# oletizi/ol_dsp

Hardware: AMD Instinct MI355X
Metric: stereo samples/s across N effect instances @48kHz; % HBM roofline; 1/2/4/8 GPU (higher is better)
Workload: dtype f32; 1 GPU; chorus; instances_per_gpu=65536, instances_total=65536, block=256, parallelism=instance-shard x1 (no data-path collective)

## Files before the change

### ol_dsp_amd/csrc/chorus_stage_rf.h

```cpp
#pragma once
#include "chorus_stage_l.h"

namespace olfx {
namespace ch {

__device__ __forceinline__ float psv_direct(Rsrc rP, uint32_t pb, uint32_t pmask, uint64_t acc, uint32_t tau,
                                            uint32_t wi, uint32_t wf, uint32_t pmaxu) {
    const uint32_t ph = hi32(acc);
    float gA, gB;
    win_gains(unit24(ph), gA, gB);
    uint32_t di; float fr;
    pitch_split(ph, wi, wf, pmaxu, di, fr);
    uint32_t q = tau - di;
    const float tA = lerp_pair(ld1(rP, pb + (q & pmask) * 8u, 0), ld1(rP, pb + ((q - 1u) & pmask) * 8u, 0), fr);
    pitch_split(ph + 0x80000000u, wi, wf, pmaxu, di, fr);
    q = tau - di;
    const float tB = lerp_pair(ld1(rP, pb + (q & pmask) * 8u, 0), ld1(rP, pb + ((q - 1u) & pmask) * 8u, 0), fr);
    return xfade(tB, gB, tA, gA);
}

template <bool COOP>
struct ChStageRF : ChStageL<false, COOP, false> {
    using B = ChStageL<false, COOP, false>;
    static constexpr int kChunk = B::kChunk, kWin = B::kWin, kSlots = B::kSlots;
    static constexpr int kTail = 12, kPsvSlots = kTail + kChunk;
    static constexpr int kSegment = 256;
    static_assert(kTail % 4 == 0, "the tail pass runs in fours");
    static constexpr int kRegion = (2 * kSlots + kPsvSlots) * kRow;
    static constexpr uint32_t kPsvWin = (uint32_t)(2 * kSlots * kRow);
    static constexpr uint32_t kOutCh = B::kOutCh;
    static_assert(B::kOutFloats <= kPsvWin && 32 * B::kStride <= (int)kPsvWin, "staging must stay below the psv window");
    static_assert(kRegion * 4 <= 20 * 1024, "two waves per SIMD");

    using B::lane; using B::j; using B::ch; using B::inst0; using B::n; using B::lfo_inc; using B::lfo_off;
    using B::ps_inc; using B::D; using B::wi; using B::wf; using B::b0; using B::b1; using B::b2; using B::a1;
    using B::a2; using B::mix; using B::dry; using B::lfo_acc; using B::ps_acc; using B::z1; using B::z2;
    using B::pmask; using B::pmaxu; using B::cmaxd; using B::rP; using B::region; using B::pl; using B::wpos;
    using B::started;

    uint32_t lead;

    __device__ __forceinline__ bool choose_lead(int len) {
        const uint64_t span = (uint64_t)(len - 1) * lfo_inc;
        const uint64_t p0 = lfo_acc + lfo_off, p1 = p0 + span;
        const bool many = lfo_inc > 0xFFFFFFFFFFFFFFFFull / (uint64_t)len;
        const bool has_max = many || p1 < p0;
        const bool has_min = many || (p1 + kHalfCycle) < (p0 + kHalfCycle);
        const float Df = (float)D, cm = (float)cmaxd;
        const float e0 = cos2pi(unit24h(p0)) * Df + Df, e1 = cos2pi(unit24h(p1)) * Df + Df;
        const float hi = fminf(fmaxf(has_max ? 2.0f * Df : fmaxf(e0, e1), 0.0f), cm);
        const float lo = fminf(fmaxf(has_min ? 0.0f : fminf(e0, e1), 0.0f), cm);
        const int dhi = min((int)(hi + 0.01f), (int)cmaxd);
        const int dlo = (int)fmaxf(lo - 0.01f, 0.0f);
        lead = (uint32_t)dlo;
        return dhi - dlo <= kTail - 1;
    }

    __device__ __forceinline__ PlanL plan_rf(uint64_t acc, int C) const {
        PlanL p;
        const uint32_t last = (uint32_t)(C - 1);
        const int L = (int)lead;
        uint32_t d0, d1;
        float fr;
        {
            const uint64_t a0 = acc, a1_ = acc + last * ps_inc;
            pitch_split(hi32(a0), wi, wf, pmaxu, d0, fr);
            pitch_split(hi32(a1_), wi, wf, pmaxu, d1, fr);
            const int lo = -(int)d1 - 1 - L, hi = (int)last - (int)d0 - L;
            p.sA = lo & ~3;
            p.okA = a1_ >= a0 && hi - p.sA < kWin;
        }
        {
            const uint64_t a0 = acc + kHalfCycle, a1_ = a0 + last * ps_inc;
            pitch_split(hi32(a0), wi, wf, pmaxu, d0, fr);
            pitch_split(hi32(a1_), wi, wf, pmaxu, d1, fr);
            const int lo = -(int)d1 - 1 - L, hi = (int)last - (int)d0 - L;
            p.sB = lo & ~3;
            p.okB = a1_ >= a0 && hi - p.sB < kWin;
        }
        p.sC = 0; p.hiC = 0;
        return p;
    }

    __device__ __forceinline__ void out_stage(int k, float v) { region[ch * kOutCh + (uint32_t)k * 32u + j] = v; }
    __device__ __forceinline__ float4 coop_out(int q) const {
        const uint32_t r = B::coop_row(q, lane);
        return *(const float4 *)(region + (r & 1u) * kOutCh + (r >> 1) * 32u + (lane & 7u) * 4u);
    }

    __device__ __forceinline__ void begin_segment(float (&x)[kChunk], int C, const float4 (&xq)[4]) {
        if (COOP) {
            B::stage_rows(xq);
            B::coop_store(true, 0, wpos, C);
            B::read_own(x, C);
        } else {
            B::stage_run(x, 0);
            B::coop_store(true, 0, wpos, C);
        }
        ps_acc -= (uint64_t)lead * ps_inc;
        float *wV = region + kPsvWin + lane;
        const uint32_t pb = B::own_pb();
#pragma unroll 1
        for (int m0 = 0; m0 < kTail; m0 += 4) {
            float tv[4];
#pragma unroll
            for (int u = 0; u < 4; ++u)
                tv[u] = psv_direct(rP, pb, pmask, ps_acc - (uint64_t)(kTail - m0 - u) * ps_inc,
                                   wpos - lead - (uint32_t)(kTail - m0 - u), wi, wf, pmaxu);
#pragma unroll
            for (int u = 0; u < 4; ++u) wV[(m0 + u) * kRow] = tv[u];
        }
        pl = plan_rf(ps_acc, C);
        started = false;
        B::template load_lines<0>(pl, wpos, true);
    }
    __device__ __forceinline__ void end_segment() { ps_acc += (uint64_t)lead * ps_inc; }

    template <int PAR>
    __device__ __forceinline__ void stores_and_next(float (&xn)[kChunk], const float4 (&xq)[4], uint32_t w0, int C,
                                                    int Cn, uint64_t ps0) {
        if (COOP) {
            if (Cn > 0) {
                B::stage_rows(xq);
                B::coop_store(true, 0, w0 + (uint32_t)C, Cn);
            }
            B::read_own(xn, Cn);
        } else if (Cn > 0) {
            B::stage_run(xn, 0);
            B::coop_store(true, 0, w0 + (uint32_t)C, Cn);
        }
        pl = plan_rf(ps0 + (uint64_t)C * ps_inc, Cn > 0 ? Cn : 4);
        B::template load_lines<PAR ^ 1>(pl, w0 + (uint32_t)C, false);
    }

    template <int PAR, class Sink, class Prefetch>
    __device__ __forceinline__ void chunk(const float (&x)[kChunk], float (&xn)[kChunk], int C, int Cn, Sink &&sink,
                                          Prefetch &&prefetch, const float4 (&xq)[4]) {
        asm volatile("" : "+v"(lane));
        j = lane >> 1;
        ch = lane & 1u;
        const uint32_t w0 = wpos;
        const uint64_t ps0 = ps_acc;
        const PlanL cur = pl;
        const int L = (int)lead;
        float psv[kChunk];
        float *wP0 = region + 0 * kSlots * kRow + lane;
        float *wP1 = region + 1 * kSlots * kRow + lane;
        float *wV = region + kPsvWin + lane;

        float tv[kTail];
        if (started) {
#pragma unroll
            for (int m = 0; m < kTail; ++m) tv[m] = wV[(kChunk + m) * kRow];
        }
        B::template stage_tap<PAR, 0>();
        B::template stage_tap<PAR, 1>();
        if (started) {
#pragma unroll
            for (int m = 0; m < kTail; ++m) wV[m * kRow] = tv[m];
        }
        {
            const int limA = kWin + cur.sA, limB = kWin + cur.sB;
            float *pA = wP0 - cur.sA * kRow, *pB = wP1 - cur.sB * kRow;
            const int mA = min(limA, C), mB = min(limB, C);
#pragma unroll
            for (int k = 0; k < kChunk; ++k) {
                pA[min(k, mA) * kRow] = x[k];
                pB[min(k, mB) * kRow] = x[k];
            }
        }
        started = true;
        __builtin_amdgcn_s_setprio(kLoadPrio);
        prefetch();
        __builtin_amdgcn_s_setprio(0);

        const bool fast = C == kChunk && __all(cur.okA && cur.okB);
        if (fast) {
            const int chA = (int)ch - L - cur.sA, chB = (int)ch - L - cur.sB;
            float gA0 = 0.f, gA1 = 0.f, gB0 = 0.f, gB1 = 0.f, fA0 = 0.f, fA1 = 0.f, fB0 = 0.f, fB1 = 0.f;
            int rA0 = 0, rA1 = 0, rB0 = 0, rB1 = 0;
#pragma unroll
            for (int k = 0; k < kChunk; ++k) {
                if ((k & 1) == 0) {
                    const uint64_t pa = ps_acc + (ch ? ps_inc : 0ull);
                    const uint32_t ph = hi32(pa);
                    float m_gA, m_gB;
                    win_gains(unit24(ph), m_gA, m_gB);
                    gA0 = pair_even(m_gA); gA1 = pair_odd(m_gA);
                    gB0 = pair_even(m_gB); gB1 = pair_odd(m_gB);
                    uint32_t di; float fr;
                    pitch_split(ph, wi, wf, pmaxu, di, fr);
                    const int ra = chA - (int)di;
                    rA0 = pair_even_i(ra); rA1 = pair_odd_i(ra);
                    fA0 = pair_even(fr); fA1 = pair_odd(fr);
                    pitch_split(ph + 0x80000000u, wi, wf, pmaxu, di, fr);
                    const int rb = chB - (int)di;
                    rB0 = pair_even_i(rb); rB1 = pair_odd_i(rb);
                    fB0 = pair_even(fr); fB1 = pair_odd(fr);
                }
                ps_acc += ps_inc;
                const bool odd = k & 1;
                const float *qA = wP0 + (k & ~1) * kRow + (odd ? rA1 : rA0) * kRow;
                const float *qB = wP1 + (k & ~1) * kRow + (odd ? rB1 : rB0) * kRow;
                const float tA = lerp_pair(qA[0], qA[-kRow], odd ? fA1 : fA0);
                const float tB = lerp_pair(qB[0], qB[-kRow], odd ? fB1 : fB0);
                psv[k] = xfade(tB, odd ? gB1 : gB0, tA, odd ? gA1 : gA0);
            }
        } else {
            const uint32_t pb = B::own_pb();
#pragma unroll 1
            for (int k0 = 0; k0 < C; k0 += 4) {
                float tv[4];
#pragma unroll
                for (int u = 0; u < 4; ++u)
                    tv[u] = psv_direct(rP, pb, pmask, ps_acc + (uint64_t)(k0 + u) * ps_inc,
                                       w0 - lead + (uint32_t)(k0 + u), wi, wf, pmaxu);
#pragma unroll
                for (int u = 0; u < 4; ++u) wV[(kTail + k0 + u) * kRow] = tv[u];
            }
            ps_acc += (uint64_t)C * ps_inc;
        }
        if (fast) {
#pragma unroll
            for (int k = 0; k < kChunk; ++k) wV[(kTail + k) * kRow] = psv[k];
        }

        stores_and_next<PAR>(xn, xq, w0, C, Cn, ps0);

        if (fast) {
            const int chC = (int)ch + kTail + L;
            int r0 = 0, r1 = 0;
            float f0 = 0.f, f1 = 0.f;
            uint32_t dn = 0;
            float fn = 0.f;
#pragma unroll
            for (int k = 0; k < kChunk; ++k) {
                if ((k & 1) == 0) {
                    uint32_t di; float fr;
                    if ((k & 3) == 0) {
                        const uint64_t p = lfo_acc + (ch ? lfo_inc : 0ull) + lfo_off;
                        chorus_split2(p, p + 2ull * lfo_inc, D, cmaxd, di, fr, dn, fn);
                    } else {
                        di = dn;
                        fr = fn;
                    }
                    const int rc = chC - (int)di;
                    r0 = pair_even_i(rc); r1 = pair_odd_i(rc);
                    f0 = pair_even(fr); f1 = pair_odd(fr);
                }
                lfo_acc += lfo_inc;
                const bool odd = k & 1;
                const float *qC = wV + (k & ~1) * kRow + (odd ? r1 : r0) * kRow;
                const float wet = lerp_pair(qC[0], qC[-kRow], odd ? f1 : f0);
                const float lp = lores_step(wet, b0, b1, b2, a1, a2, z1, z2);
                sink(k, dry_wet(x[k], dry, lp, mix));
            }
        } else {
#pragma unroll
            for (int k = 0; k < kChunk; ++k) {
                if (k >= C) continue;
                uint32_t di; float fr;
                chorus_split(lfo_acc + lfo_off, D, cmaxd, di, fr);
                lfo_acc += lfo_inc;
                const int jw = kTail + k + L - (int)di;
                const float wet = lerp_pair(wV[jw * kRow], wV[(jw - 1) * kRow], fr);
                const float lp = lores_step(wet, b0, b1, b2, a1, a2, z1, z2);
                sink(k, dry_wet(x[k], dry, lp, mix));
            }
        }
        wpos = w0 + (uint32_t)C;
    }
};

}
}
```

Baseline: 99.44 billion stereo samples/s.

## Compute segment lead-in tail via staged window lines instead of direct ring loads

```diff
diff --git a/ol_dsp_amd/csrc/chorus_stage_rf.h b/ol_dsp_amd/csrc/chorus_stage_rf.h
--- a/ol_dsp_amd/csrc/chorus_stage_rf.h
+++ b/ol_dsp_amd/csrc/chorus_stage_rf.h
@@ -39,6 +39,12 @@
     using B::started;
 
     uint32_t lead;
+    Rsrc rNone;
+
+    __device__ __forceinline__ void init(const ChorusArgs &a, float *lds_region, uint32_t lane_, uint32_t inst0_) {
+        B::init(a, lds_region, lane_, inst0_);
+        rNone = rsrc(a.pitch_ring, 0);
+    }
 
     __device__ __forceinline__ bool choose_lead(int len) {
         const uint64_t span = (uint64_t)(len - 1) * lfo_inc;
@@ -88,7 +94,48 @@
         return *(const float4 *)(region + (r & 1u) * kOutCh + (r >> 1) * 32u + (lane & 7u) * 4u);
     }
 
+    template <int K0>
+    __device__ __forceinline__ void phase_a(uint64_t &acc, const PlanL &p, const float *wP0, const float *wP1,
+                                            float (&psv)[kChunk]) const {
+        static_assert(K0 % 2 == 0, "frame pairs");
+        const int L = (int)lead;
+        const int chA = (int)ch - L - p.sA, chB = (int)ch - L - p.sB;
+        float gA0 = 0.f, gA1 = 0.f, gB0 = 0.f, gB1 = 0.f, fA0 = 0.f, fA1 = 0.f, fB0 = 0.f, fB1 = 0.f;
+        int rA0 = 0, rA1 = 0, rB0 = 0, rB1 = 0;
+#pragma unroll
+        for (int k = K0; k < kChunk; ++k) {
+            if ((k & 1) == 0) {
+                const uint64_t pa = acc + (ch ? ps_inc : 0ull);
+                const uint32_t ph = hi32(pa);
+                float m_gA, m_gB;
+                win_gains(unit24(ph), m_gA, m_gB);
+                gA0 = pair_even(m_gA); gA1 = pair_odd(m_gA);
+                gB0 = pair_even(m_gB); gB1 = pair_odd(m_gB);
+                uint32_t di; float fr;
+                pitch_split(ph, wi, wf, pmaxu, di, fr);
+                const int ra = chA - (int)di;
+                rA0 = pair_even_i(ra); rA1 = pair_odd_i(ra);
+                fA0 = pair_even(fr); fA1 = pair_odd(fr);
+                pitch_split(ph + 0x80000000u, wi, wf, pmaxu, di, fr);
+                const int rb = chB - (int)di;
+                rB0 = pair_even_i(rb); rB1 = pair_odd_i(rb);
+                fB0 = pair_even(fr); fB1 = pair_odd(fr);
+            }
+            acc += ps_inc;
+            const bool odd = k & 1;
+            const float *qA = wP0 + (k & ~1) * kRow + (odd ? rA1 : rA0) * kRow;
+            const float *qB = wP1 + (k & ~1) * kRow + (odd ? rB1 : rB0) * kRow;
+            const float tA = lerp_pair(qA[0], qA[-kRow], odd ? fA1 : fA0);
+            const float tB = lerp_pair(qB[0], qB[-kRow], odd ? fB1 : fB0);
+            psv[k] = xfade(tB, odd ? gB1 : gB0, tA, odd ? gA1 : gA0);
+        }
+    }
+
     __device__ __forceinline__ void begin_segment(float (&x)[kChunk], int C, const float4 (&xq)[4]) {
+        ps_acc -= (uint64_t)lead * ps_inc;
+        const PlanL li = plan_rf(ps_acc - (uint64_t)kChunk * ps_inc, kChunk);
+        const bool leadin = __all(li.okA && li.okB);
+        if (leadin) B::template load_lines<1>(li, wpos - (uint32_t)kChunk, true);
         if (COOP) {
             B::stage_rows(xq);
             B::coop_store(true, 0, wpos, C);
@@ -97,22 +144,33 @@
             B::stage_run(x, 0);
             B::coop_store(true, 0, wpos, C);
         }
-        ps_acc -= (uint64_t)lead * ps_inc;
         float *wV = region + kPsvWin + lane;
-        const uint32_t pb = B::own_pb();
+        if (leadin) {
+            B::template stage_tap<1, 0>();
+            B::template stage_tap<1, 1>();
+        } else {
+            const uint32_t pb = B::own_pb();
 #pragma unroll 1
-        for (int m0 = 0; m0 < kTail; m0 += 4) {
-            float tv[4];
-#pragma unroll
-            for (int u = 0; u < 4; ++u)
-                tv[u] = psv_direct(rP, pb, pmask, ps_acc - (uint64_t)(kTail - m0 - u) * ps_inc,
-                                   wpos - lead - (uint32_t)(kTail - m0 - u), wi, wf, pmaxu);
-#pragma unroll
-            for (int u = 0; u < 4; ++u) wV[(m0 + u) * kRow] = tv[u];
+            for (int m0 = 0; m0 < kTail; m0 += 4) {
+                float tv[4];
+#pragma unroll
+                for (int u = 0; u < 4; ++u)
+                    tv[u] = psv_direct(rP, pb, pmask, ps_acc - (uint64_t)(kTail - m0 - u) * ps_inc,
+                                       wpos - lead - (uint32_t)(kTail - m0 - u), wi, wf, pmaxu);
+#pragma unroll
+                for (int u = 0; u < 4; ++u) wV[(m0 + u) * kRow] = tv[u];
+            }
         }
         pl = plan_rf(ps_acc, C);
         started = false;
-        B::template load_lines<0>(pl, wpos, true);
+        B::template load_lines<0>(pl, wpos, !leadin);
+        if (leadin) {
+            float psv[kChunk];
+            uint64_t acc = ps_acc - (uint64_t)kTail * ps_inc;
+            phase_a<kChunk - kTail>(acc, li, region + 0 * kSlots * kRow + lane, region + 1 * kSlots * kRow + lane, psv);
+#pragma unroll
+            for (int m = 0; m < kTail; ++m) wV[m * kRow] = psv[kChunk - kTail + m];
+        }
     }
     __device__ __forceinline__ void end_segment() { ps_acc += (uint64_t)lead * ps_inc; }
 
@@ -130,7 +188,10 @@
             B::coop_store(true, 0, w0 + (uint32_t)C, Cn);
         }
         pl = plan_rf(ps0 + (uint64_t)C * ps_inc, Cn > 0 ? Cn : 4);
+        const Rsrc ring = rP;
+        rP = Cn > 0 ? ring : rNone;
         B::template load_lines<PAR ^ 1>(pl, w0 + (uint32_t)C, false);
+        rP = ring;
     }
 
     template <int PAR, class Sink, class Prefetch>
@@ -176,36 +237,7 @@
 
         const bool fast = C == kChunk && __all(cur.okA && cur.okB);
         if (fast) {
-            const int chA = (int)ch - L - cur.sA, chB = (int)ch - L - cur.sB;
-            float gA0 = 0.f, gA1 = 0.f, gB0 = 0.f, gB1 = 0.f, fA0 = 0.f, fA1 = 0.f, fB0 = 0.f, fB1 = 0.f;
-            int rA0 = 0, rA1 = 0, rB0 = 0, rB1 = 0;
-#pragma unroll
-            for (int k = 0; k < kChunk; ++k) {
-                if ((k & 1) == 0) {
-                    const uint64_t pa = ps_acc + (ch ? ps_inc : 0ull);
-                    const uint32_t ph = hi32(pa);
-                    float m_gA, m_gB;
-                    win_gains(unit24(ph), m_gA, m_gB);
-                    gA0 = pair_even(m_gA); gA1 = pair_odd(m_gA);
-                    gB0 = pair_even(m_gB); gB1 = pair_odd(m_gB);
-                    uint32_t di; float fr;
-                    pitch_split(ph, wi, wf, pmaxu, di, fr);
-                    const int ra = chA - (int)di;
-                    rA0 = pair_even_i(ra); rA1 = pair_odd_i(ra);
-                    fA0 = pair_even(fr); fA1 = pair_odd(fr);
-                    pitch_split(ph + 0x80000000u, wi, wf, pmaxu, di, fr);
-                    const int rb = chB - (int)di;
-                    rB0 = pair_even_i(rb); rB1 = pair_odd_i(rb);
-                    fB0 = pair_even(fr); fB1 = pair_odd(fr);
-                }
-                ps_acc += ps_inc;
-                const bool odd = k & 1;
-                const float *qA = wP0 + (k & ~1) * kRow + (odd ? rA1 : rA0) * kRow;
-                const float *qB = wP1 + (k & ~1) * kRow + (odd ? rB1 : rB0) * kRow;
-                const float tA = lerp_pair(qA[0], qA[-kRow], odd ? fA1 : fA0);
-                const float tB = lerp_pair(qB[0], qB[-kRow], odd ? fB1 : fB0);
-                psv[k] = xfade(tB, odd ? gB1 : gB0, tA, odd ? gA1 : gA0);
-            }
+            phase_a<0>(ps_acc, cur, wP0, wP1, psv);
         } else {
             const uint32_t pb = B::own_pb();
 #pragma unroll 1
```

Result: faster. 103.3 billion stereo samples/s, median of 6 (+3.9%).
